# CVLAB-Unibo/MM2D3D

Hardware: AMD Instinct MI355X
Metric: LiDAR scenes/sec fwd+bwd (NuScenes ~35k pts, 5cm voxel) (higher is better)
Workload: dtype fp16 MFMA, fp32 accumulate, loss scale 65536 on the device (2D branch: IEEE fp16 maps and packed weights - the reference's precision: 16 = fp16 autocast + GradScaler) + f32 (3D sparse branch, fp32 as in the reference: f32 MFMA on narrow layers, fp32-faithful 3-term split-bf16 products with fp32 accu; 1 GPU; BASELINE.json configs[1]: NuScenes-shaped (32x1090 sweep, 34,880 pts/scene), 5 cm voxels, 480x302 RGB + sparse depth; full two-domain training step (train.py:186-292): 2D+3D fwd on source and target, 2 CE + 4 KL, backward, AdamW x2 + OneCycle; distinct_batches_rotated=4, parallelism=dp1

## Files before the change

include/mm2d3d.h:

```cpp
#ifndef MM2D3D_H
#define MM2D3D_H

#include <stddef.h>
#include <stdint.h>

#ifdef __cplusplus
extern "C" {
#endif

typedef void* mm_stream_t;

#define MM_OK 0
#define MM_ERR_ARG (-1)
#define MM_ERR_HIP (-2)
#define MM_ERR_WORKSPACE (-3)
#define MM_ERR_UNSUPPORTED (-4)

const char* mm_last_error(void);

typedef void* mm_handle_t;
size_t mm_handle_sync_bytes(void);
size_t mm_handle_fault_bytes(void);
int mm_create(int device_id, void* sync_dev, size_t sync_bytes, void* fault_host, size_t fault_bytes, mm_handle_t* out);
int mm_destroy(mm_handle_t h);
// ... 233 lines not shown
int mm_rmsprop_step(float* p, const float* g, float* sq, float* gavg, float* buf, int64_t n, double lr, double alpha, double eps,
                    double weight_decay, double momentum, double grad_scale, const int* skip_dev, int nskip, mm_stream_t stream);
int mm_sgd_prepare(const float* scale_dev, const int* found_dev, int nfound, int64_t* step_dev, int advance, double lr,
                   double momentum, double dampening, double weight_decay, double grad_scale, void* coef_dev, mm_stream_t stream);
int mm_adam_prepare(const float* scale_dev, const int* found_dev, int nfound, int64_t* step_dev, int advance, double lr,
                    double beta1, double beta2, double eps, double weight_decay, int decoupled, double grad_scale, void* coef_dev,
                    mm_stream_t stream);
int mm_rmsprop_prepare(const float* scale_dev, const int* found_dev, int nfound, int64_t* step_dev, int advance, double lr,
                       double alpha, double eps, double weight_decay, double momentum, double grad_scale, void* coef_dev,
                       mm_stream_t stream);
int mm_sgd_step_dev(float* p, const float* g, float* buf, int64_t n, int nesterov, const void* coef_dev, mm_stream_t stream);
int mm_adam_step_dev(float* p, const float* g, float* m, float* v, float* vmax, int64_t n, int decoupled, const void* coef_dev,
                     mm_stream_t stream);
int mm_rmsprop_step_dev(float* p, const float* g, float* sq, float* gavg, float* buf, int64_t n, const void* coef_dev,
                        mm_stream_t stream);

int mm_ema_row_bytes(void);
int mm_ema_update(const void* table_dev, int nrows, int64_t nblocks, double decay, int warmup, int64_t t_host, const int64_t* step_dev,
                  const void* coef_dev, const int* skip_dev, int nskip, mm_stream_t stream);
int mm_ema_swap(const void* table_dev, int nrows, int64_t nblocks, mm_stream_t stream);

size_t mm_grad_sqnorm_ws_bytes(int64_t n);
int mm_grad_sqnorm(const float* g, int64_t n, void* partial_ws, int64_t slot, int* found_dev, mm_stream_t stream);
int mm_clip_finalize(const void* partial_ws, const int64_t* counts, int narenas, const float* scale_dev, double grad_scale,
                     double max_norm, float* norm_out_dev, float* eff_scale_out_dev, mm_stream_t stream);
int mm_grad_clip_value(float* g, int64_t n, double clip_value, const float* scale_dev, double grad_scale, mm_stream_t stream);

int mm_conv2d_gemm(const void* A, int B, int Hi, int Wi, int Ca, int lda, void* O, int Ho, int Wo, int Cn, int ldo,
                   int out_f32, int Hg, int Wg, int so, int ooy, int oox, int sa, int fr, int ntaps, const int* ty,
                   const int* tx, const void* Wp, int nz, int64_t wz, int zpar, const float* bias, float* stats,
                   int64_t split_m, const void* addend, int ld_add, mm_stream_t stream);
int mm_conv2d_dgrad_s2(const void* dY, int B, int Ho, int Wo, int Cout, int ldy, void* dX, int H, int W, int Cin, int ldx, const void* Wd,
                       int k, int pad, const void* addend, int ld_add, mm_stream_t stream);
int64_t mm_conv2d_gemm_stat_rows(int64_t M, int nz);
int64_t mm_conv2d_3x3s1_stat_rows(int B, int H, int W);
int mm_conv2d_3x3s1(const void* A, int B, int H, int W, int Ca, int lda, void* O, int Cn, int ldo, const void* Wp,
                    const float* bias, int flip, float* stats, int split_b, mm_stream_t stream);
int mm_conv2d_3x3s1_pair(const void* A0, const void* A1, int B, int H, int W, int Ca, int lda, void* O0, void* O1, int Cn, int ldo,
                         const void* Wp0, const void* Wp1, int flip, float* stats0, float* stats1, int split_b, mm_stream_t stream);
size_t mm_conv2d_wgrad_ws_bytes(int64_t M, int Cn, int Ck, int ntaps);
int mm_conv2d_wgrad(const void* X, int B, int Hi, int Wi, int Ck, int ldx, const void* dY, int Hg, int Wg, int Cn,
                    int ldy, int sa, int ntaps, const int* ty, const int* tx, float* dW, int64_t sn, int64_t st,
                    int64_t sk, int accumulate, void* ws, size_t ws_bytes, mm_stream_t stream);
int mm_conv2d_wgrad3x3_pair(const void* X0, const void* X1, int B, int H, int W, int Ck, int ldx, const void* dY0, const void* dY1, int Cn,
                            int ldy, float* dW0, float* dW1, int64_t sn, int64_t st, int64_t sk, int accumulate, void* ws, size_t ws_bytes,
                            mm_stream_t stream);
int mm_conv2d_wgrad_slabs(const void* X, int B, int Hi, int Wi, int Ck, int ldx, const void* dY, int Hg, int Wg, int Cn, int ldy,
                          int sa, int ntaps, const int* ty, const int* tx, void* slabs, size_t slab_bytes, int* nsplit,
                          mm_stream_t stream);
int mm_conv2d_wgrad3x3_pair_slabs(const void* X0, const void* X1, int B, int H, int W, int Ck, int ldx, const void* dY0, const void* dY1,
                                  int Cn, int ldy, void* slabs, size_t slab_bytes, int* nsplit, mm_stream_t stream);
int mm_conv2d_wgrad_reduce_desc_bytes(void);
int64_t mm_conv2d_wgrad_reduce_blocks(int Cn, int Ck, int pair);
int mm_conv2d_wgrad_reduce_batch(const void* descs_dev, int n, int64_t total_blocks, mm_stream_t stream);
int64_t mm_conv2d_stem7_stat_rows(int B, int H, int W);
int mm_conv2d_stem7(const void* xb, int B, int Hb, int Wb, int H, int W, int R, int T, void* O, int ldo, const void* Wp, float* stats,
                    int split_b, mm_stream_t stream);
int mm_stem_prep(const float* in, int B, int C, int H, int W, int pad, int Hb, int Wb, int R, void* out, mm_stream_t stream);
int mm_pack_weights_bf16(const float* in, void* out, int Z, int N, int T, int K, int64_t sz, int64_t sn, int64_t st,
                         int64_t sk, mm_stream_t stream);
int mm_pack_weights_bf16_batch(const int64_t* desc, int ndesc, int64_t total_blocks, mm_stream_t stream);

size_t mm_bn2d_ws_bytes(int C);
int mm_bn2d_fwd_train(mm_handle_t h, const void* x, int ld_x, const void* res, int ld_r, int64_t N, int64_t Ns, int C, const float* weight,
                      const float* bias, float* running_mean, float* running_var, int64_t* num_batches_tracked, float eps,
                      float momentum, int relu, void* y, int ld_y, float* save_mean, float* save_invstd, void* ws,
// ... 31 lines not shown
                int ld_dx, void* dres, int ld_dr, float* dweight, float* dbias, int accumulate, void* ws, size_t ws_bytes,
                mm_stream_t stream);

int mm_colsum_bf16(const void* x, int ld_x, int64_t N, int C, float* out, int accumulate, void* ws, size_t ws_bytes,
                   mm_stream_t stream);

int mm_copy_rows_bf16(const void* src, int64_t ld_s, void* dst, int64_t ld_d, int64_t N, int C, mm_stream_t stream);
int mm_concat_bf16(void* const* parts, const int* channels, int nparts, void* wide, int64_t N, int split, mm_stream_t stream);
int mm_maxpool3x3s2_fwd(const void* x, int ldx, int B, int H, int W, int C, void* y, void* idx, mm_stream_t stream);
int mm_maxpool3x3s2_bwd(const void* dy, int ld_dy, const void* dy2, int ld_dy2, const void* idx, int B, int H, int W, int C, void* dx,
                        mm_stream_t stream);
size_t mm_head_ws_bytes(int B, int h, int w, int Hp, int Wp, int C, int NJ);
int mm_head_fwd(const void* x, int B, int Hp, int Wp, int ld, int h, int w, int C, const float* Wj, const float* bias,
                int NJ, float* out, void* ws, size_t ws_bytes, mm_stream_t stream);
int mm_head_bwd(const void* x, int B, int Hp, int Wp, int ld, int h, int w, int C, const float* Wj, int NJ,
                const float* dout, void* dx, float* dWj, void* ws, size_t ws_bytes, mm_stream_t stream);

int mm_conv2d_f32(const float* A, int B, int Hi, int Wi, int Ca, int ldA, float* O, int Ho, int Wo, int Cn, int ldO, int KH, int KW,
                  int so, int sgn, int off, int up, const float* W, int64_t w_sn, int64_t w_sc, int64_t w_sy, int64_t w_sx,
                  const float* bias, mm_stream_t stream);
size_t mm_conv2d_f32_wgrad_ws_bytes(int64_t n_pixels, int Cg, int Ca, int KH, int KW);
int mm_conv2d_f32_wgrad(const float* G, int B, int Hg, int Wg, int Cg, int ldG, const float* A, int Hi, int Wi, int Ca, int ldA,
                        int KH, int KW, int so, int sgn, int off, int up, float* dW, int64_t w_sn, int64_t w_sc, int64_t w_sy,
                        int64_t w_sx, int accumulate, void* ws, size_t ws_bytes, mm_stream_t stream);
int mm_colsum_f32(const float* x, int ld, int64_t N, int C, float* out, int accumulate, mm_stream_t stream);


int mm_conv2d_gemm_f16(const void* A, int B, int Hi, int Wi, int Ca, int lda, void* O, int Ho, int Wo, int Cn, int ldo,
                   int out_f32, int Hg, int Wg, int so, int ooy, int oox, int sa, int fr, int ntaps, const int* ty,
                   const int* tx, const void* Wp, int nz, int64_t wz, int zpar, const float* bias, float* stats,
                   int64_t split_m, const void* addend, int ld_add, mm_stream_t stream);
int mm_conv2d_dgrad_s2_f16(const void* dY, int B, int Ho, int Wo, int Cout, int ldy, void* dX, int H, int W, int Cin, int ldx, const void* Wd,
                       int k, int pad, const void* addend, int ld_add, mm_stream_t stream);
int64_t mm_conv2d_gemm_stat_rows_f16(int64_t M, int nz);
int64_t mm_conv2d_3x3s1_stat_rows_f16(int B, int H, int W);
int mm_conv2d_3x3s1_f16(const void* A, int B, int H, int W, int Ca, int lda, void* O, int Cn, int ldo, const void* Wp,
                    const float* bias, int flip, float* stats, int split_b, mm_stream_t stream);
int mm_conv2d_3x3s1_pair_f16(const void* A0, const void* A1, int B, int H, int W, int Ca, int lda, void* O0, void* O1, int Cn, int ldo,
                         const void* Wp0, const void* Wp1, int flip, float* stats0, float* stats1, int split_b, mm_stream_t stream);
int mm_conv2d_wgrad3x3_pair_f16(const void* X0, const void* X1, int B, int H, int W, int Ck, int ldx, const void* dY0, const void* dY1, int Cn,
                            int ldy, float* dW0, float* dW1, int64_t sn, int64_t st, int64_t sk, int accumulate, void* ws, size_t ws_bytes,
                            mm_stream_t stream);
size_t mm_conv2d_wgrad_ws_bytes_f16(int64_t M, int Cn, int Ck, int ntaps);
int mm_conv2d_wgrad_f16(const void* X, int B, int Hi, int Wi, int Ck, int ldx, const void* dY, int Hg, int Wg, int Cn,
                    int ldy, int sa, int ntaps, const int* ty, const int* tx, float* dW, int64_t sn, int64_t st,
                    int64_t sk, int accumulate, void* ws, size_t ws_bytes, mm_stream_t stream);
int mm_conv2d_wgrad_slabs_f16(const void* X, int B, int Hi, int Wi, int Ck, int ldx, const void* dY, int Hg, int Wg, int Cn, int ldy,
                          int sa, int ntaps, const int* ty, const int* tx, void* slabs, size_t slab_bytes, int* nsplit,
                          mm_stream_t stream);
int mm_conv2d_wgrad3x3_pair_slabs_f16(const void* X0, const void* X1, int B, int H, int W, int Ck, int ldx, const void* dY0, const void* dY1,
                                  int Cn, int ldy, void* slabs, size_t slab_bytes, int* nsplit, mm_stream_t stream);
int mm_conv2d_wgrad_reduce_desc_bytes_f16(void);
int64_t mm_conv2d_wgrad_reduce_blocks_f16(int Cn, int Ck, int pair);
int mm_conv2d_wgrad_reduce_batch_f16(const void* descs_dev, int n, int64_t total_blocks, mm_stream_t stream);
int64_t mm_conv2d_stem7_stat_rows_f16(int B, int H, int W);
int mm_conv2d_stem7_f16(const void* xb, int B, int Hb, int Wb, int H, int W, int R, int T, void* O, int ldo, const void* Wp, float* stats,
                    int split_b, mm_stream_t stream);
int mm_stem_prep_f16(const float* in, int B, int C, int H, int W, int pad, int Hb, int Wb, int R, void* out, mm_stream_t stream);
int mm_pack_weights_f16(const float* in, void* out, int Z, int N, int T, int K, int64_t sz, int64_t sn, int64_t st,
                         int64_t sk, mm_stream_t stream);
int mm_pack_weights_f16_batch(const int64_t* desc, int ndesc, int64_t total_blocks, mm_stream_t stream);
size_t mm_bn2d_ws_bytes_f16(int C);
int mm_bn2d_fwd_train_f16(mm_handle_t h, const void* x, int ld_x, const void* res, int ld_r, int64_t N, int64_t Ns, int C, const float* weight,
                      const float* bias, float* running_mean, float* running_var, int64_t* num_batches_tracked, float eps,
                      float momentum, int relu, void* y, int ld_y, float* save_mean, float* save_invstd, void* ws,
                      size_t ws_bytes, mm_stream_t stream);
// ... 39 lines not shown
```

mm2d3d_amd/_lib.py:

```python
from __future__ import annotations

import contextlib
import ctypes as C
import os
import subprocess

import torch

_HERE = os.path.dirname(os.path.abspath(__file__))
LIB_PATH = os.environ.get("MM_LIB_PATH") or os.path.join(_HERE, "libmm2d3d_hip.so")
CSRC = os.path.join(_HERE, "csrc")

_lib = None

vp, i32, i64, sz, f32, f64 = C.c_void_p, C.c_int32, C.c_int64, C.c_size_t, C.c_float, C.c_double

_PROTOS = {
    "mm_last_error": (C.c_char_p, []),
    "mm_handle_sync_bytes": (sz, []),
    "mm_handle_fault_bytes": (sz, []),
    "mm_create": (i32, [i32, vp, sz, vp, sz, C.POINTER(vp)]),
    "mm_destroy": (i32, [vp]),
    "mm_set_option": (i32, [vp, i32, i32]),
    "mm_get_option": (i32, [vp, i32]),
# ... 80 lines not shown
    "mm_lift_index_ws_bytes": (sz, [i64]),
    "mm_lift_index": (i32, [vp, vp, i32, i64, i32, i32, i32, vp, vp, vp, vp, vp, sz, vp]),
    "mm_lift_gather_key": (i32, [vp, i64, i64, i64, i64, vp, i64, i32, i32, i32, vp, vp]),
    "mm_lift_scatter_key": (i32, [vp, i32, vp, vp, i64, i32, i32, i64, i64, i64, i64, vp, vp]),
    "mm_eval_confusion": (i32, [vp, i32, vp, i32, vp, i64, i32, i64, vp, vp]),
    "mm_pselab_predict": (i32, [vp, i32, vp, i32, i64, i32, vp, vp, vp, vp, vp, vp, vp]),
    "mm_teacher_labels": (i32, [vp, i32, vp, i32, i64, i32, i32, f32, i64, vp, vp, vp, vp, vp, vp]),
    "mm_pselab_refine_ws_bytes": (sz, [i32]),
    "mm_pselab_refine": (i32, [vp, vp, i64, i32, i64, vp, vp, sz, vp]),
    "mm_grad_nonfinite": (i32, [vp, i64, vp, vp]),
    "mm_amp_update": (i32, [vp, vp, vp, i32, f64, f64, i32, vp]),
    "mm_optim_coef_bytes": (i32, []),
    "mm_sgd_step": (i32, [vp, vp, vp, i64, f64, f64, f64, f64, i32, i64, f64, vp, i32, vp]),
    "mm_adam_step": (i32, [vp, vp, vp, vp, vp, i64, f64, f64, f64, f64, f64, i32, i64, f64, vp, i32, vp]),
    "mm_rmsprop_step": (i32, [vp, vp, vp, vp, vp, i64, f64, f64, f64, f64, f64, f64, vp, i32, vp]),
    "mm_sgd_prepare": (i32, [vp, vp, i32, vp, i32, f64, f64, f64, f64, f64, vp, vp]),
    "mm_adam_prepare": (i32, [vp, vp, i32, vp, i32, f64, f64, f64, f64, f64, i32, f64, vp, vp]),
    "mm_rmsprop_prepare": (i32, [vp, vp, i32, vp, i32, f64, f64, f64, f64, f64, f64, vp, vp]),
    "mm_sgd_step_dev": (i32, [vp, vp, vp, i64, i32, vp, vp]),
    "mm_adam_step_dev": (i32, [vp, vp, vp, vp, vp, i64, i32, vp, vp]),
    "mm_rmsprop_step_dev": (i32, [vp, vp, vp, vp, vp, i64, vp, vp]),
    "mm_ema_row_bytes": (i32, []),
    "mm_ema_update": (i32, [vp, i32, i64, f64, i32, i64, vp, vp, vp, i32, vp]),
    "mm_ema_swap": (i32, [vp, i32, i64, vp]),
    "mm_grad_sqnorm_ws_bytes": (sz, [i64]),
    "mm_grad_sqnorm": (i32, [vp, i64, vp, i64, vp, vp]),
    "mm_clip_finalize": (i32, [vp, vp, i32, vp, f64, f64, vp, vp, vp]),
    "mm_grad_clip_value": (i32, [vp, i64, f64, vp, f64, vp]),
    "mm_conv2d_gemm": (i32, [vp, i32, i32, i32, i32, i32, vp, i32, i32, i32, i32, i32, i32, i32, i32, i32, i32, i32, i32, i32, vp, vp,
                             vp, i32, i64, i32, vp, vp, i64, vp, i32, vp]),
    "mm_conv2d_3x3s1": (i32, [vp, i32, i32, i32, i32, i32, vp, i32, i32, vp, vp, i32, vp, i32, vp]),
    "mm_conv2d_3x3s1_pair": (i32, [vp, vp, i32, i32, i32, i32, i32, vp, vp, i32, i32, vp, vp, i32, vp, vp, i32, vp]),
    "mm_conv2d_dgrad_s2": (i32, [vp, i32, i32, i32, i32, i32, vp, i32, i32, i32, i32, vp, i32, i32, vp, i32, vp]),
    "mm_conv2d_gemm_stat_rows": (i64, [i64, i32]),
    "mm_conv2d_3x3s1_stat_rows": (i64, [i32, i32, i32]),
    "mm_conv2d_wgrad_ws_bytes": (sz, [i64, i32, i32, i32]),
    "mm_conv2d_wgrad": (i32, [vp, i32, i32, i32, i32, i32, vp, i32, i32, i32, i32, i32, i32, vp, vp, vp, i64, i64, i64, i32, vp, sz,
                              vp]),
    "mm_conv2d_wgrad3x3_pair": (i32, [vp, vp, i32, i32, i32, i32, i32, vp, vp, i32, i32, vp, vp, i64, i64, i64, i32, vp, sz, vp]),
    "mm_conv2d_wgrad_slabs": (i32, [vp, i32, i32, i32, i32, i32, vp, i32, i32, i32, i32, i32, i32, vp, vp, vp, sz, vp, vp]),
    "mm_conv2d_wgrad3x3_pair_slabs": (i32, [vp, vp, i32, i32, i32, i32, i32, vp, vp, i32, i32, vp, sz, vp, vp]),
    "mm_conv2d_wgrad_reduce_desc_bytes": (i32, []),
    "mm_conv2d_wgrad_reduce_blocks": (i64, [i32, i32, i32]),
    "mm_conv2d_wgrad_reduce_batch": (i32, [vp, i32, i64, vp]),
    "mm_conv2d_f32": (i32, [vp, i32, i32, i32, i32, i32, vp, i32, i32, i32, i32, i32, i32, i32, i32, i32, i32, vp, i64, i64, i64, i64, vp, vp]),
    "mm_conv2d_f32_wgrad_ws_bytes": (sz, [i64, i32, i32, i32, i32]),
    "mm_conv2d_f32_wgrad": (i32, [vp, i32, i32, i32, i32, i32, vp, i32, i32, i32, i32, i32, i32, i32, i32, i32, i32, vp, i64, i64, i64, i64,
                                  i32, vp, sz, vp]),
    "mm_colsum_f32": (i32, [vp, i32, i64, i32, vp, i32, vp]),
    "mm_pack_weights_bf16": (i32, [vp, vp, i32, i32, i32, i32, i64, i64, i64, i64, vp]),
    "mm_pack_weights_bf16_batch": (i32, [vp, i32, i64, vp]),
    "mm_conv2d_stem7_stat_rows": (i64, [i32, i32, i32]),
    "mm_conv2d_stem7": (i32, [vp, i32, i32, i32, i32, i32, i32, i32, vp, i32, vp, vp, i32, vp]),
    "mm_stem_prep": (i32, [vp, i32, i32, i32, i32, i32, i32, i32, i32, vp, vp]),
    "mm_bn2d_ws_bytes": (sz, [i32]),
    "mm_bn2d_fwd_train": (i32, [vp, vp, i32, vp, i32, i64, i64, i32, vp, vp, vp, vp, vp, f32, f32, i32, vp, i32, vp, vp, vp, sz, vp]),
    "mm_bn2d_single_launch": (i32, [vp, i64, i64, i32, i32]),
    "mm_bn2d_fwd_train_pre": (i32, [vp, i32, vp, i32, i64, i64, i32, vp, vp, vp, vp, vp, f32, f32, i32, vp, i32, vp, vp, vp, i64, vp, sz, vp]),
    "mm_bn2d_fwd_train_pre_pool": (i32, [vp, i32, i32, i32, i32, i32, i32, vp, vp, vp, vp, vp, f32, f32, vp, i32, vp, vp, vp, vp, vp, i64, vp, sz, vp]),
    "mm_bn2d_bwd_pool": (i32, [vp, i32, vp, i32, vp, i32, i32, i32, i32, vp, i32, i32, vp, vp, vp, vp, vp, i32, vp, vp, i32, vp, sz, vp]),
    "mm_bn2d_fwd_train_pair": (i32, [vp, vp, vp, i64, i64, i32, f32, f32, i32, vp, sz, vp]),
    "mm_bn2d_bwd_pair": (i32, [vp, vp, vp, i32, i64, i64, i32, i32, vp, sz, vp]),
    "mm_bn2d_fwd_eval": (i32, [vp, i32, vp, i32, i64, i32, vp, vp, vp, vp, f32, i32, vp, i32, vp]),
    "mm_bn2d_bwd": (i32, [vp, vp, i32, vp, i32, vp, i32, vp, i32, i32, i64, i64, i32, vp, vp, vp, vp, vp, i32, vp, i32, vp, vp, i32, vp, sz, vp]),
    "mm_colsum_bf16": (i32, [vp, i32, i64, i32, vp, i32, vp, sz, vp]),
    "mm_copy_rows_bf16": (i32, [vp, i64, vp, i64, i64, i32, vp]),
    "mm_concat_bf16": (i32, [vp, vp, i32, vp, i64, i32, vp]),
    "mm_maxpool3x3s2_fwd": (i32, [vp, i32, i32, i32, i32, i32, vp, vp, vp]),
    "mm_maxpool3x3s2_bwd": (i32, [vp, i32, vp, i32, vp, i32, i32, i32, i32, vp, vp]),
    "mm_head_ws_bytes": (sz, [i32, i32, i32, i32, i32, i32, i32]),
    "mm_head_fwd": (i32, [vp, i32, i32, i32, i32, i32, i32, i32, vp, vp, i32, vp, vp, sz, vp]),
    "mm_head_bwd": (i32, [vp, i32, i32, i32, i32, i32, i32, i32, vp, i32, vp, vp, vp, vp, sz, vp]),
}


class Bn2dFwdArgs(C.Structure):
    _fields_ = [("x", C.c_void_p), ("ld_x", C.c_int), ("res", C.c_void_p), ("ld_r", C.c_int), ("weight", C.c_void_p), ("bias", C.c_void_p),
                ("running_mean", C.c_void_p), ("running_var", C.c_void_p), ("num_batches_tracked", C.c_void_p), ("y", C.c_void_p),
                ("ld_y", C.c_int), ("save_mean", C.c_void_p), ("save_invstd", C.c_void_p)]


class Bn2dBwdArgs(C.Structure):
    _fields_ = [("x", C.c_void_p), ("ld_x", C.c_int), ("dy", C.c_void_p), ("ld_dy", C.c_int), ("dy2", C.c_void_p), ("ld_dy2", C.c_int),
                ("yout", C.c_void_p), ("ld_y", C.c_int), ("weight", C.c_void_p), ("bias", C.c_void_p), ("save_mean", C.c_void_p),
                ("save_invstd", C.c_void_p), ("dx", C.c_void_p), ("ld_dx", C.c_int), ("dres", C.c_void_p), ("ld_dr", C.c_int),
                ("dweight", C.c_void_p), ("dbias", C.c_void_p)]


class HipLibraryMissing(RuntimeError):
    pass


H16_2D = {
    "mm_conv2d_gemm": "mm_conv2d_gemm_f16",
    "mm_conv2d_dgrad_s2": "mm_conv2d_dgrad_s2_f16",
    "mm_conv2d_3x3s1": "mm_conv2d_3x3s1_f16",
    "mm_conv2d_3x3s1_pair": "mm_conv2d_3x3s1_pair_f16",
    "mm_conv2d_gemm_stat_rows": "mm_conv2d_gemm_stat_rows_f16",
    "mm_conv2d_3x3s1_stat_rows": "mm_conv2d_3x3s1_stat_rows_f16",
    "mm_bn2d_fwd_train_pre": "mm_bn2d_fwd_train_pre_f16",
    "mm_bn2d_single_launch": "mm_bn2d_single_launch_f16",
    "mm_bn2d_fwd_train_pair": "mm_bn2d_fwd_train_pair_f16",
    "mm_bn2d_fwd_train_pre_pool": "mm_bn2d_fwd_train_pre_pool_f16",
    "mm_bn2d_bwd_pool": "mm_bn2d_bwd_pool_f16",
    "mm_bn2d_bwd_pair": "mm_bn2d_bwd_pair_f16",
    "mm_conv2d_wgrad_ws_bytes": "mm_conv2d_wgrad_ws_bytes_f16",
    "mm_conv2d_wgrad": "mm_conv2d_wgrad_f16",
    "mm_conv2d_wgrad3x3_pair": "mm_conv2d_wgrad3x3_pair_f16",
    "mm_conv2d_wgrad_slabs": "mm_conv2d_wgrad_slabs_f16",
    "mm_conv2d_wgrad3x3_pair_slabs": "mm_conv2d_wgrad3x3_pair_slabs_f16",
    "mm_conv2d_wgrad_reduce_desc_bytes": "mm_conv2d_wgrad_reduce_desc_bytes_f16",
    "mm_conv2d_wgrad_reduce_blocks": "mm_conv2d_wgrad_reduce_blocks_f16",
    "mm_conv2d_wgrad_reduce_batch": "mm_conv2d_wgrad_reduce_batch_f16",
    "mm_stem_prep": "mm_stem_prep_f16",
    "mm_conv2d_stem7_stat_rows": "mm_conv2d_stem7_stat_rows_f16",
    "mm_conv2d_stem7": "mm_conv2d_stem7_f16",
    "mm_pack_weights_bf16": "mm_pack_weights_f16",
    "mm_pack_weights_bf16_batch": "mm_pack_weights_f16_batch",
    "mm_bn2d_ws_bytes": "mm_bn2d_ws_bytes_f16",
    "mm_bn2d_fwd_train": "mm_bn2d_fwd_train_f16",
    "mm_bn2d_fwd_eval": "mm_bn2d_fwd_eval_f16",
    "mm_bn2d_bwd": "mm_bn2d_bwd_f16",
    "mm_colsum_bf16": "mm_colsum_f16",
    "mm_maxpool3x3s2_fwd": "mm_maxpool3x3s2_fwd_f16",
    "mm_maxpool3x3s2_bwd": "mm_maxpool3x3s2_bwd_f16",
    "mm_head_ws_bytes": "mm_head_ws_bytes_f16",
    "mm_head_fwd": "mm_head_fwd_f16",
    "mm_head_bwd": "mm_head_bwd_f16",
}
for _a, _b in H16_2D.items():
# ... 206 lines not shown
```

mm2d3d_amd/conv2d.py:

```python
from __future__ import annotations

import ctypes as C
import os
import weakref

import torch

from . import _lib, domains, gradsink
from ._lib import check, ptr, stream

CL = torch.channels_last

WHOLE_ITEMS = [2 if os.environ.get("MM_CONV_WHOLE_ITEMS", "0") != "0" else 0]
LEGACY3X3 = [{"1": 4, "2": 8, "3": 12}.get(os.environ.get("MM_CONV3X3_LEGACY", "0"), 0)]
BN_PRE = [{"0": False, "1": True}.get(os.environ.get("MM_BN2D_PRE", "auto"), "auto")]
WGRAD_BATCH = [os.environ.get("MM_CONV_WGRAD_BATCH", "1") != "0"]
WGRAD_BATCH_GRAPH = [os.environ.get("MM_CONV_WGRAD_BATCH_GRAPH", "1") != "0"]
STEM7 = [os.environ.get("MM_CONV_STEM7", "1") != "0"]
DGRAD_S2 = [os.environ.get("MM_CONV_DGRAD_S2", "1") != "0"]
PAIR = [os.environ.get("MM_CONV_PAIR", "1") != "0"]
PAIR_WGRAD = [os.environ.get("MM_CONV_PAIR_WGRAD", "1") != "0"]

HALF = [torch.float16]


def set_half(dtype):
    if dtype not in (torch.bfloat16, torch.float16):
        raise ValueError("the 16-bit storage format of the 2D branch is torch.bfloat16 or torch.float16")
    HALF[0] = dtype


class _Lib2d:

    def __getattr__(self, name):
        L = _lib.lib()
        if HALF[0] == torch.float16:
            alt = _lib.H16_2D.get(name)
            if alt is not None:
                return getattr(L, alt)
        return getattr(L, name)


_LIB2D = _Lib2d()


def lib2d():
    return _LIB2D


def nhwc_pitch(x):
    if x.dtype != HALF[0]:
        x = x.to(HALF[0])
    B, C, H, W = x.shape
    s0, s1, s2, s3 = x.stride()
    if s1 == 1 and s3 >= C and s3 % 8 == 0 and s2 == W * s3 and s0 == H * W * s3 and x.data_ptr() % 16 == 0:
        return x, s3
    return x.contiguous(memory_format=CL), C


def _arr(v):
    return (C.c_int * len(v))(*v)


def as_nhwc_bf16(x):
    if x.dtype != HALF[0]:
        x = x.to(HALF[0])
    if not x.is_contiguous(memory_format=CL):
        x = x.contiguous(memory_format=CL)
# ... 535 lines not shown
```

mm2d3d_amd/csrc/conv2d.hip:

```cpp
#include <hip/hip_bf16.h>

#include <type_traits>

#include "common.h"
#include "h16.h"

typedef h16x8 bf16x8;
typedef short s16x4 __attribute__((ext_vector_type(4)));
typedef float f32x16 __attribute__((ext_vector_type(16)));

namespace {

constexpr int MAXT = 16;

struct ConvP {
  const u16* A;
  int B, Hi, Wi, Ca, lda;
  void* O;
  int Ho, Wo, Cn, ldo;
  int Hg, Wg;
  int so, ooy, oox;
  int sa, fr;
  int ntaps;
  short ty[MAXT], tx[MAXT];
// ... 295 lines not shown
    }
#pragma unroll
    for (int j = 0; j < TN; j++) {
#pragma unroll
      for (int q = 0; q < 4; q++) {
        const int n = n0 + wn * (BN / 2) + j * 32 + 8 * q + 4 * fh;
        if (n >= p.Cn) continue;
        float v[4];
#pragma unroll
        for (int e = 0; e < 4; e++) v[e] = acc[i][j][4 * q + e];
        if (vec) {
          if (p.bias) {
            const float4 bb = *(const float4*)&p.bias[n];
            v[0] += bb.x, v[1] += bb.y, v[2] += bb.z, v[3] += bb.w;
          }
          if (p.out_f32) {
            *(float4*)&((float*)p.O)[orow * p.ldo + n] = make_float4(v[0], v[1], v[2], v[3]);
          } else {
            uint2 o;
            o.x = (unsigned)f2bf(v[0]) | ((unsigned)f2bf(v[1]) << 16);
            o.y = (unsigned)f2bf(v[2]) | ((unsigned)f2bf(v[3]) << 16);
            *(uint2*)&((u16*)p.O)[orow * p.ldo + n] = o;
          }
        } else {
#pragma unroll
          for (int e = 0; e < 4; e++)
            if (n + e < p.Cn) {
              const float w = v[e] + (p.bias ? p.bias[n + e] : 0.f);
              if (p.out_f32)
                ((float*)p.O)[orow * p.ldo + n + e] = w;
              else
                ((u16*)p.O)[orow * p.ldo + n + e] = f2bf(w);
            }
        }
      }
    }
  }
}

struct C3P {
  const u16* A;
  int B, H, W, Ca, lda;
  u16* O;
  int Cn, ldo;
  const u16* Wp;
  const float* bias;
  int flip;
  int whole;
  int legacy;
  float* stats;
  int split_b;
  int tiles_y, tiles_x;
  int B1;
  const u16* A1;
  u16* O1;
  const u16* Wp1;
  float* stats1;
};
#define MM_DIAG(p, bit) ((DIAG & (bit)) != 0)

__device__ __attribute__((aligned(16))) unsigned int g_dump[256];


#ifdef MM_DIAG_CLOCK
__device__ unsigned long long g_clk[3][1024][2];
#define MM_CLK_BEGIN() const unsigned long long clk_t0 = __builtin_amdgcn_s_memtime(), clk_r0 = __builtin_amdgcn_s_memrealtime()
// ... 1975 lines not shown
    const int sy = y + r - pad, sx = x - pad;
    v[sl] = (r < R && sy >= 0 && sy < H && sx >= 0 && sx < W) ? f2bf(in[((int64_t)(b * C + c) * H + sy) * W + sx]) : (u16)0;
  }
  unsigned w[4];
#pragma unroll
  for (int i = 0; i < 4; i++) w[i] = (unsigned)v[2 * i] | ((unsigned)v[2 * i + 1] << 16);
  *(uint4*)(out + (int64_t)gid * 8) = make_uint4(w[0], w[1], w[2], w[3]);
}

int fill_taps(ConvP* p, const int* ty, const int* tx, int nt) {
  if (nt > MAXT) return -1;
  p->ntaps = nt;
  p->wtaps = nt;
  p->zwin = 0;
  for (int i = 0; i < nt; i++) {
    p->ty[i] = (short)ty[i];
    p->tx[i] = (short)tx[i];
    p->wt[i] = (short)i;
  }
  for (int i = 0; i < 4; i++) p->zt0[i] = p->znt[i] = 0;
  return 0;
}

}

extern "C" {

#ifdef MM_DIAG_CLOCK
int MM_SYM(mm_diag_clock_read)(void* out_host, size_t bytes) {
  return hipMemcpyFromSymbol(out_host, HIP_SYMBOL(g_clk), bytes < sizeof(g_clk) ? bytes : sizeof(g_clk)) == hipSuccess ? 0 : -1;
}
#endif

static int gemm_launch(ConvP p, int nz, int steps_max, hipStream_t s) {
  const int B = p.B, Hg = p.Hg, Wg = p.Wg, Cn = p.Cn;
  const int64_t M = (int64_t)B * Hg * Wg;
  if (M == 0) return MM_OK;
  MM_CHECK_ARG(M < (1ll << 31), "conv2d_gemm: too many output pixels for 32-bit pixel indices");
  {
    constexpr int single_max = 4;
    p.nbuf = (steps_max <= single_max && (Cn <= 64 || steps_max == 1)) ? 1 : 2;
  }
  if (Cn <= 64) {
    size_t lds = (size_t)p.nbuf * (128 * 64 + 64 * 64) * 2;
    hipLaunchKernelGGL(k_conv_gemm<64>, dim3((unsigned)mm_cdiv(M, 128), (unsigned)mm_cdiv(Cn, 64), nz), dim3(256), lds, s, p);
  } else {
    size_t lds = (size_t)p.nbuf * (128 * 64 + 128 * 64) * 2;
    static unsigned once = 0;
    if (mm_attr_todo(&once)) {
      MM_HIP(hipFuncSetAttribute((const void*)k_conv_gemm<128>, hipFuncAttributeMaxDynamicSharedMemorySize, (int)(2 * (128 * 64 + 128 * 64) * 2)));
      mm_attr_done(&once);
    }
    hipLaunchKernelGGL(k_conv_gemm<128>, dim3((unsigned)mm_cdiv(M, 128), (unsigned)mm_cdiv(Cn, 128), nz), dim3(256), lds, s, p);
  }
  MM_LAUNCH_CHECK();
  return MM_OK;
}

int MM_SYM(mm_conv2d_gemm)(const void* A, int B, int Hi, int Wi, int Ca, int lda, void* O, int Ho, int Wo, int Cn, int ldo,
                   int out_f32, int Hg, int Wg, int so, int ooy, int oox, int sa, int fr, int ntaps, const int* ty,
                   const int* tx, const void* Wp, int nz, int64_t wz, int zpar, const float* bias, float* stats, int64_t split_m,
                   const void* addend, int ld_add, hipStream_t s) {
  MM_CHECK_ARG(Ca % 64 == 0 && lda % 8 == 0 && ((uintptr_t)A % 16) == 0 && ((uintptr_t)Wp % 16) == 0,
               "conv2d_gemm: Ca must be a multiple of 64 and pointers 16-B aligned (Ca=%d lda=%d)", Ca, lda);
  MM_CHECK_ARG(!stats || (!out_f32 && Cn % 32 == 0 && ldo % 8 == 0 && ((uintptr_t)O % 16) == 0 && ((uintptr_t)bias % 16) == 0),
               "conv2d_gemm: statistics need a 16-bit output, Cn a multiple of 32, ldo of 8");
  MM_CHECK_ARG(!addend || (!out_f32 && Cn % 8 == 0 && ldo % 8 == 0 && ld_add % 8 == 0 && ((uintptr_t)O % 16) == 0 && ((uintptr_t)addend % 16) == 0 &&
                           ((uintptr_t)bias % 16) == 0),
               "conv2d_gemm: an addend needs a 16-bit output, channels and pitches multiples of 8, 16-byte aligned maps");
  MM_CHECK_ARG(fr == 1 || fr == 2, "conv2d_gemm: fr must be 1 or 2");
  ConvP p;
// ... 437 lines not shown
```

Before: 486.1 scenes/s.

## Add persistent weight-resident conv GEMM kernel with double-buffered activation tiles

Adds a persistent-grid conv GEMM kernel that loads the whole packed weight matrix into LDS once per workgroup and then loops over 128-row output tiles. Activation chunks are double-buffered with global_load_lds, and the next tile's first chunk is prefetched during the epilogue. It also folds the four transposed-conv sub-positions into one wide N tile and handles the stride-2 1x1 dgrad zero fill inside the same kernel. The path is on by default for eligible shapes. It trades higher LDS use, and possibly lower occupancy, for fewer weight reloads and fewer launch tails.

```diff
diff --git a/include/mm2d3d.h b/include/mm2d3d.h
--- a/include/mm2d3d.h
+++ b/include/mm2d3d.h
@@ -289,6 +289,7 @@
                    int64_t split_m, const void* addend, int ld_add, mm_stream_t stream);
 int mm_conv2d_dgrad_s2(const void* dY, int B, int Ho, int Wo, int Cout, int ldy, void* dX, int H, int W, int Cin, int ldx, const void* Wd,
                        int k, int pad, const void* addend, int ld_add, mm_stream_t stream);
+int mm_conv2d_gemm_rw(int mode, int wgs);
 int64_t mm_conv2d_gemm_stat_rows(int64_t M, int nz);
 int64_t mm_conv2d_3x3s1_stat_rows(int B, int H, int W);
 int mm_conv2d_3x3s1(const void* A, int B, int H, int W, int Ca, int lda, void* O, int Cn, int ldo, const void* Wp,
@@ -386,6 +387,7 @@
                    int64_t split_m, const void* addend, int ld_add, mm_stream_t stream);
 int mm_conv2d_dgrad_s2_f16(const void* dY, int B, int Ho, int Wo, int Cout, int ldy, void* dX, int H, int W, int Cin, int ldx, const void* Wd,
                        int k, int pad, const void* addend, int ld_add, mm_stream_t stream);
+int mm_conv2d_gemm_rw_f16(int mode, int wgs);
 int64_t mm_conv2d_gemm_stat_rows_f16(int64_t M, int nz);
 int64_t mm_conv2d_3x3s1_stat_rows_f16(int B, int H, int W);
 int mm_conv2d_3x3s1_f16(const void* A, int B, int H, int W, int Ca, int lda, void* O, int Cn, int ldo, const void* Wp,
diff --git a/mm2d3d_amd/_lib.py b/mm2d3d_amd/_lib.py
--- a/mm2d3d_amd/_lib.py
+++ b/mm2d3d_amd/_lib.py
@@ -136,6 +136,7 @@
     "mm_conv2d_3x3s1": (i32, [vp, i32, i32, i32, i32, i32, vp, i32, i32, vp, vp, i32, vp, i32, vp]),
     "mm_conv2d_3x3s1_pair": (i32, [vp, vp, i32, i32, i32, i32, i32, vp, vp, i32, i32, vp, vp, i32, vp, vp, i32, vp]),
     "mm_conv2d_dgrad_s2": (i32, [vp, i32, i32, i32, i32, i32, vp, i32, i32, i32, i32, vp, i32, i32, vp, i32, vp]),
+    "mm_conv2d_gemm_rw": (i32, [i32, i32]),
     "mm_conv2d_gemm_stat_rows": (i64, [i64, i32]),
     "mm_conv2d_3x3s1_stat_rows": (i64, [i32, i32, i32]),
     "mm_conv2d_wgrad_ws_bytes": (sz, [i64, i32, i32, i32]),
@@ -200,6 +201,7 @@
     "mm_conv2d_dgrad_s2": "mm_conv2d_dgrad_s2_f16",
     "mm_conv2d_3x3s1": "mm_conv2d_3x3s1_f16",
     "mm_conv2d_3x3s1_pair": "mm_conv2d_3x3s1_pair_f16",
+    "mm_conv2d_gemm_rw": "mm_conv2d_gemm_rw_f16",
     "mm_conv2d_gemm_stat_rows": "mm_conv2d_gemm_stat_rows_f16",
     "mm_conv2d_3x3s1_stat_rows": "mm_conv2d_3x3s1_stat_rows_f16",
     "mm_bn2d_fwd_train_pre": "mm_bn2d_fwd_train_pre_f16",
diff --git a/mm2d3d_amd/conv2d.py b/mm2d3d_amd/conv2d.py
--- a/mm2d3d_amd/conv2d.py
+++ b/mm2d3d_amd/conv2d.py
@@ -30,10 +30,26 @@
     HALF[0] = dtype
 
 
+GEMM_RW = [(1 if os.environ.get("MM_CONV_GEMM_RW", "1") != "0" else 0) | (2 if os.environ.get("MM_CONV_GEMM_RW_DEBUG", "0") != "0" else 0), 0]
+_GEMM_RW_SENT = [False]
+
+
+def set_gemm_rw(mode, wgs=0):
+    prev = tuple(GEMM_RW)
+    GEMM_RW[0], GEMM_RW[1] = int(mode), int(wgs)
+    L = _lib.lib()
+    check(L.mm_conv2d_gemm_rw(GEMM_RW[0], GEMM_RW[1]), "conv2d_gemm_rw")
+    check(L.mm_conv2d_gemm_rw_f16(GEMM_RW[0], GEMM_RW[1]), "conv2d_gemm_rw")
+    _GEMM_RW_SENT[0] = True
+    return prev
+
+
 class _Lib2d:
 
     def __getattr__(self, name):
         L = _lib.lib()
+        if not _GEMM_RW_SENT[0]:
+            set_gemm_rw(*GEMM_RW)
         if HALF[0] == torch.float16:
             alt = _lib.H16_2D.get(name)
             if alt is not None:
diff --git a/mm2d3d_amd/csrc/conv2d.hip b/mm2d3d_amd/csrc/conv2d.hip
--- a/mm2d3d_amd/csrc/conv2d.hip
+++ b/mm2d3d_amd/csrc/conv2d.hip
@@ -351,6 +351,254 @@
               else
                 ((u16*)p.O)[orow * p.ldo + n + e] = f2bf(w);
             }
+        }
+      }
+    }
+  }
+}
+
+struct RwP {
+  ConvP c;
+  int fold;
+  int dz;
+  int steps;
+  int ntiles;
+  int tyx[8];
+};
+
+template <int TN>
+__global__ __launch_bounds__(256, 2) void k_conv_gemm_rw(RwP q) {
+  const ConvP& p = q.c;
+  extern __shared__ __attribute__((aligned(16))) u16 smem[];
+  constexpr int NT = TN * 64;
+  u16* Bs = smem;
+  u16* As = smem + q.steps * NT * 64;
+  float* Bias = (float*)(As + 2 * 128 * 64);
+  const int tid = threadIdx.x, wave = tid >> 6, lane = tid & 63;
+  const int wm = wave >> 1, wn = wave & 1;
+  const int64_t M = (int64_t)p.B * p.Hg * p.Wg;
+  const int cc = tid & 7, r0 = tid >> 3;
+  const int kcn = p.Ca >> 6;
+
+  for (int s = 0; s < q.steps; s++) {
+    const int tl = s / kcn, kc = s - tl * kcn;
+    const int woff = p.wt[tl] * p.Ca + kc * 64;
+#pragma unroll
+    for (int i = 0; i < NT / 32; i++) {
+      const int row = r0 + 32 * i;
+      const u16* g = p.W + (int64_t)row * p.wtaps * p.Ca + woff + ((cc ^ ((row >> 1) & 7)) << 3);
+      __builtin_amdgcn_global_load_lds((const __attribute__((address_space(1))) void*)g,
+                                       (__attribute__((address_space(3))) void*)(Bs + s * NT * 64 + (wave * 8 + 32 * i) * 64), 16, 0, 0);
+    }
+  }
+
+  const u16* abase[4];
+  unsigned amask[4];
+  auto decode = [&](int tile) {
+    const int64_t m0 = (int64_t)tile * 128;
+#pragma unroll
+    for (int i = 0; i < 4; i++) {
+      const int row = r0 + 32 * i;
+      const int64_t m = m0 + row;
+      int ab = -1, ay = 0, ax = 0;
+      if (m < M) {
+        const unsigned mu = (unsigned)m, t = mu / (unsigned)p.Wg;
+        ax = (int)(mu - t * (unsigned)p.Wg);
+        ab = (int)(t / (unsigned)p.Hg);
+        ay = (int)(t - (unsigned)ab * (unsigned)p.Hg);
+      }
+      abase[i] = p.A + ((int64_t)((ab < 0 ? 0 : ab) * p.Hi + ay * p.sa) * p.Wi + ax * p.sa) * p.lda + ((cc ^ ((row >> 1) & 7)) << 3);
+      unsigned mk = 0;
+      if (ab >= 0)
+        for (int t = 0; t < p.ntaps; t++) {
+          const int v = q.tyx[t];
+          const int sy = ay * p.sa + (short)(v & 0xffff), sx = ax * p.sa + (v >> 16);
+          if (sy >= 0 && sx >= 0 && sy < p.Hi && sx < p.Wi) mk |= 1u << t;
+        }
+      amask[i] = mk;
+    }
+  };
+  auto issue = [&](int s, int buf) {
+    const int tap = s / kcn, kc = s - tap * kcn;
+    const int v = q.tyx[tap];
+    const int64_t toff = ((int64_t)(short)(v & 0xffff) * p.Wi + (v >> 16)) * p.lda + kc * 64;
+#pragma unroll
+    for (int i = 0; i < 4; i++) {
+      const u16* g = (amask[i] >> tap) & 1u ? abase[i] + toff : (const u16*)g_zero16;
+      __builtin_amdgcn_global_load_lds((const __attribute__((address_space(1))) void*)g,
+                                       (__attribute__((address_space(3))) void*)(As + buf * 128 * 64 + (wave * 8 + 32 * i) * 64), 16, 0, 0);
+    }
+  };
+
+  const int fr_ = lane & 31, fh = lane >> 5;
+  const int schunk = frag_chunk(lane);
+  const bool remap = p.so != 1 || p.Ho != p.Hg || p.Wo != p.Wg;
+  int tile = blockIdx.x;
+  if (tile >= q.ntiles) return;
+  decode(tile);
+  issue(0, 0);
+  if (p.bias && tid < NT) Bias[tid] = p.bias[q.fold ? tid & 63 : tid];
+  __syncthreads();
+  unsigned g = 0;
+  constexpr int NST = 4 * TN;
+  bool stores_behind = false;
+  for (; tile < q.ntiles; tile += gridDim.x) {
+    f32x16 acc[2][TN];
+#pragma unroll
+    for (int i = 0; i < 2; i++)
+#pragma unroll
+      for (int j = 0; j < TN; j++)
+#pragma unroll
+        for (int r = 0; r < 16; r++) acc[i][j][r] = 0.f;
+
+    for (int s = 0; s < q.steps; s++, g++) {
+      const int buf = g & 1;
+      if (s == 0 && stores_behind)
+        asm volatile("s_waitcnt vmcnt(%0)\n\ts_barrier" ::"n"(NST) : "memory");
+      else
+        asm volatile("s_waitcnt vmcnt(0)\n\ts_barrier" ::: "memory");
+      if (s + 1 < q.steps) {
+        issue(s + 1, buf ^ 1);
+      } else if (tile + (int)gridDim.x < q.ntiles) {
+        decode(tile + gridDim.x);
+        issue(0, buf ^ 1);
+      }
+      const u16* Ab = As + buf * 128 * 64;
+      const u16* Bb = Bs + s * NT * 64;
+#pragma unroll
+      for (int kk = 0; kk < 4; kk++) {
+        bf16x8 af[2], bf[TN];
+        const int ch = kk * 2 + fh;
+#pragma unroll
+        for (int i = 0; i < 2; i++) {
+          int row = wm * 64 + i * 32 + fr_;
+          af[i] = *(const bf16x8*)&Ab[row * 64 + ((ch ^ ((row >> 1) & 7)) << 3)];
+        }
+#pragma unroll
+        for (int j = 0; j < TN; j++) {
+          int row = wn * (NT / 2) + j * 32 + fr_;
+          bf[j] = *(const bf16x8*)&Bb[row * 64 + ((ch ^ ((row >> 1) & 7)) << 3)];
+        }
+#pragma unroll
+        for (int i = 0; i < 2; i++)
+#pragma unroll
+          for (int j = 0; j < TN; j++) acc[i][j] = MM_MFMA_32x32x16(bf[j], af[i], acc[i][j]);
+      }
+    }
+
+    const int64_t m0 = (int64_t)tile * 128;
+    stores_behind = m0 + 128 <= M;
+    int ora[2], orb[2], mra[2], mrb[2];
+#pragma unroll
+    for (int i = 0; i < 2; i++) {
+      mra[i] = (int)m0 + wm * 64 + i * 32 + (lane & 15), mrb[i] = mra[i] + 16;
+      auto out_row = [&](int m) -> int {
+        if (remap) {
+          const unsigned mu = (unsigned)m, t = mu / (unsigned)p.Wg;
+          const int gx = (int)(mu - t * (unsigned)p.Wg);
+          const int b = (int)(t / (unsigned)p.Hg), gy = (int)(t - (unsigned)b * (unsigned)p.Hg);
+          return (b * p.Ho + gy * p.so) * p.Wo + gx * p.so;
+        }
+        return m;
+      };
+      ora[i] = mra[i] < M ? out_row(mra[i]) : -1;
+      orb[i] = mrb[i] < M ? out_row(mrb[i]) : -1;
+    }
+#pragma unroll
+    for (int j = 0; j < TN; j++) {
+      uint4 sxa[2], sxb[2];
+      const int ntot = wn * (NT / 2) + j * 32;
+      const int zf = q.fold ? ntot >> 6 : 0;
+      const int nf = q.fold ? ntot & 63 : ntot;
+      const int zoff = (zf >> 1) * p.Wo + (zf & 1);
+      const int64_t ssub = ((int64_t)zf * q.ntiles + tile) * 2 + wm;
+      typedef float f32x4 __attribute__((ext_vector_type(4)));
+      f32x4 bq[4] = {};
+      const unsigned ba = (unsigned)(uintptr_t)(__attribute__((address_space(3))) float*)&Bias[ntot + 4 * fh];
+      if (TN < 4 && p.bias) {
+        asm volatile("ds_read_b128 %0, %4\n\tds_read_b128 %1, %4 offset:32\n\tds_read_b128 %2, %4 offset:64\n\tds_read_b128 %3, %4 offset:96\n\t"
+                     "s_waitcnt lgkmcnt(0)"
+                     : "=&v"(bq[0]), "=&v"(bq[1]), "=&v"(bq[2]), "=&v"(bq[3])
+                     : "v"(ba));
+      }
+      constexpr bool ADD = TN < 4;
+      uint4 ada[2], adb[2];
+      if (ADD && p.addend) {
+#pragma unroll
+        for (int i = 0; i < 2; i++) {
+          ada[i] = *(const uint4*)(p.addend + (ora[i] >= 0 ? (int64_t)(ora[i] + zoff) * p.ld_add : 0) + nf + 8 * schunk);
+          adb[i] = *(const uint4*)(p.addend + (orb[i] >= 0 ? (int64_t)(orb[i] + zoff) * p.ld_add : 0) + nf + 8 * schunk);
+        }
+      }
+#pragma unroll
+      for (int i = 0; i < 2; i++) {
+        unsigned D[4][2];
+#pragma unroll
+        for (int qd = 0; qd < 4; qd++) {
+          float v[4];
+#pragma unroll
+          for (int e = 0; e < 4; e++) v[e] = acc[i][j][4 * qd + e];
+          if (p.bias) {
+            f32x4 bb;
+            if constexpr (TN < 4) bb = bq[qd];
+            else asm volatile("ds_read_b128 %0, %1\n\ts_waitcnt lgkmcnt(0)" : "=v"(bb) : "v"(ba + 32 * qd));
+            v[0] += bb.x, v[1] += bb.y, v[2] += bb.z, v[3] += bb.w;
+          }
+          D[qd][0] = (unsigned)f2bf(v[0]) | ((unsigned)f2bf(v[1]) << 16);
+          D[qd][1] = (unsigned)f2bf(v[2]) | ((unsigned)f2bf(v[3]) << 16);
+        }
+        uint4 xa, xb;
+        frag_rows(D, xa, xb);
+        const int n = nf + 8 * schunk;
+        u16* rowa = ora[i] >= 0 ? (u16*)p.O + (int64_t)(ora[i] + zoff) * p.ldo : nullptr;
+        u16* rowb = orb[i] >= 0 ? (u16*)p.O + (int64_t)(orb[i] + zoff) * p.ldo : nullptr;
+        if (ADD && p.addend) {
+          if (rowa) xa = add_h8(xa, ada[i]);
+          if (rowb) xb = add_h8(xb, adb[i]);
+        }
+        sxa[i] = xa, sxb[i] = xb;
+        if (rowa) *(uint4*)(rowa + n) = xa;
+        if (rowb) *(uint4*)(rowb + n) = xb;
+      }
+      if (p.stats) {
+#pragma unroll
+        for (int grp = 0; grp < 2; grp++) {
+          float st[16];
+#pragma unroll
+          for (int t = 0; t < 16; t++) st[t] = 0.f;
+#pragma unroll
+          for (int i = 0; i < 2; i++) {
+            stats_accum(sxa[i], ora[i] >= 0 && (mra[i] < p.split_m) == (grp == 0), st);
+            stats_accum(sxb[i], orb[i] >= 0 && (mrb[i] < p.split_m) == (grp == 0), st);
+          }
+          stats_store(p.stats, 2 * ssub + grp, p.Cn, nf, lane, row_reduce_scatter16(st, lane & 15), false);
+        }
+      }
+    }
+    if (TN < 4 && q.dz) {
+      for (int z = 1; z < 4; z++) {
+        const int zoff = (z >> 1) * p.Wo + (z & 1);
+#pragma unroll
+        for (int j = 0; j < TN; j++) {
+          const int n = wn * (NT / 2) + j * 32 + 8 * schunk;
+          uint4 ada[2], adb[2];
+          if (p.addend) {
+#pragma unroll
+            for (int i = 0; i < 2; i++) {
+              ada[i] = *(const uint4*)(p.addend + (ora[i] >= 0 ? (int64_t)(ora[i] + zoff) * p.ld_add : 0) + n);
+              adb[i] = *(const uint4*)(p.addend + (orb[i] >= 0 ? (int64_t)(orb[i] + zoff) * p.ld_add : 0) + n);
+            }
+          }
+#pragma unroll
+          for (int i = 0; i < 2; i++) {
+            uint4 xa = make_uint4(0u, 0u, 0u, 0u), xb = xa;
+            if (p.addend) {
+              xa = add_h8(xa, ada[i]);
+              xb = add_h8(xb, adb[i]);
+            }
+            if (ora[i] >= 0) *(uint4*)((u16*)p.O + (int64_t)(ora[i] + zoff) * p.ldo + n) = xa;
+            if (orb[i] >= 0) *(uint4*)((u16*)p.O + (int64_t)(orb[i] + zoff) * p.ldo + n) = xb;
+          }
         }
       }
     }
@@ -2392,11 +2640,93 @@
 }
 #endif
 
+static int g_rw_mode = 1, g_rw_wgs = 0;
+int MM_SYM(mm_conv2d_gemm_rw)(int mode, int wgs) {
+  MM_CHECK_ARG(mode >= 0 && mode < 8 && wgs >= 0, "conv2d_gemm_rw: mode is 0..7, wgs >= 0");
+  __atomic_store_n(&g_rw_mode, mode, __ATOMIC_RELAXED);
+  __atomic_store_n(&g_rw_wgs, wgs, __ATOMIC_RELAXED);
+  return MM_OK;
+}
+
+static int rw_launch(const ConvP& p, int nz, hipStream_t s, int* done) {
+  *done = 0;
+  const int mode = __atomic_load_n(&g_rw_mode, __ATOMIC_RELAXED), wgs_forced = __atomic_load_n(&g_rw_wgs, __ATOMIC_RELAXED);
+  if (!(mode & 1)) return MM_OK;
+  const int64_t M = (int64_t)p.B * p.Hg * p.Wg;
+  RwP q;
+  q.c = p;
+  q.fold = q.dz = 0;
+  int nt_eff = p.ntaps;
+  if (nz == 4 && p.zpar && !p.zwin) {
+    if (p.ntaps != 1 || p.Cn != 64 || p.wz != (int64_t)p.Cn * p.Ca || p.so != 2) return MM_OK;
+    q.fold = 1;
+  } else if (nz == 4 && p.zpar && p.zwin) {
+    if (p.znt[0] != 1 || p.zt0[0] != 0 || p.znt[1] || p.znt[2] || p.znt[3] || p.ntaps != 1 || p.so != 2 || p.Cn > 128) return MM_OK;
+    q.dz = 1;
+    nt_eff = 1;
+  } else if (nz != 1 || p.zwin) {
+    return MM_OK;
+  }
+  const int NT = q.fold ? 4 * p.Cn : p.Cn;
+  q.steps = nt_eff * (p.Ca / 64);
+  if (p.out_f32 || p.fr != 1 || p.ooy || p.oox || (p.Cn & 63) || (p.ldo & 7) || p.lda < p.Ca || p.ldo < p.Cn || ((uintptr_t)p.O & 15) ||
+      ((uintptr_t)p.bias & 15) || (p.addend && ((p.ld_add & 7) || p.ld_add < p.Cn || ((uintptr_t)p.addend & 15))))
+    return MM_OK;
+  if ((NT != 64 && NT != 128 && NT != 256) || q.steps < 1 || (int64_t)NT * q.steps * 64 > 32768) return MM_OK;
+  if (NT == 256 && p.addend) return MM_OK;
+  if ((int64_t)p.B * p.Hi * p.Wi >= (1ll << 31) || (int64_t)p.B * p.Ho * p.Wo >= (1ll << 31)) return MM_OK;
+  q.ntiles = (int)mm_cdiv(M, 128);
+  static const int ncu = [] {
+    int dev = 0, n = 0;
+    if (hipGetDevice(&dev) != hipSuccess || hipDeviceGetAttribute(&n, hipDeviceAttributeMultiprocessorCount, dev) != hipSuccess || n <= 0) n = 256;
+    return n;
+  }();
+  for (int t = 0; t < 8; t++) q.tyx[t] = t < p.ntaps ? (int)(((unsigned)p.ty[t] & 0xffffu) | ((unsigned)p.tx[t] << 16)) : 0;
+  const size_t lds = ((size_t)q.steps * NT * 64 + 2 * 128 * 64) * 2 + (size_t)NT * 4;
+  const int per_cu = lds <= 66560 ? 2 : 1;
+  if (wgs_forced <= 0 && !(mode & 4) && per_cu == 1 && !q.fold) return MM_OK;
+  int wgs = wgs_forced > 0 ? wgs_forced : per_cu * ncu;
+  if (wgs > q.ntiles) wgs = q.ntiles;
+  for (int e = 0; e < 2; e++) {
+    const int64_t m = e ? M - 1 : 0;
+    const int ax = (int)(m % p.Wg), ay = (int)(m / p.Wg % p.Hg), ab = (int)(m / p.Wg / p.Hg);
+    for (int t = 0; t < nt_eff; t++) {
+      const int sy = ay * p.sa + p.ty[t], sx = ax * p.sa + p.tx[t];
+      if (sy < 0 || sx < 0 || sy >= p.Hi || sx >= p.Wi) continue;
+      const int64_t px = ((int64_t)ab * p.Hi + sy) * p.Wi + sx;
+      MM_CHECK_ARG(ab >= 0 && ab < p.B && px >= 0 && px < (int64_t)p.B * p.Hi * p.Wi, "conv2d_gemm_rw: a source pixel outside the input map");
+    }
+  }
+  static unsigned once = 0;
+  if (mm_attr_todo(&once)) {
+    const int mx = (32768 + 2 * 128 * 64) * 2 + 256 * 4;
+    MM_HIP(hipFuncSetAttribute((const void*)k_conv_gemm_rw<1>, hipFuncAttributeMaxDynamicSharedMemorySize, mx));
+    MM_HIP(hipFuncSetAttribute((const void*)k_conv_gemm_rw<2>, hipFuncAttributeMaxDynamicSharedMemorySize, mx));
+    MM_HIP(hipFuncSetAttribute((const void*)k_conv_gemm_rw<4>, hipFuncAttributeMaxDynamicSharedMemorySize, mx));
+    mm_attr_done(&once);
+  }
+  if (mode & 2)
+    fprintf(stderr, "conv2d_gemm_rw: K=%d N=%d %s M=%lld tiles=%d wgs=%d lds=%zu addend=%d stats=%d\n", q.steps * 64, NT,
+            q.fold ? "convT-fwd" : q.dz ? "dgrad-s2-1x1" : p.sa == 2 ? "gather-s2" : "plain", (long long)M, q.ntiles, wgs, lds,
+            p.addend != nullptr, p.stats != nullptr);
+  if (NT == 64) hipLaunchKernelGGL(k_conv_gemm_rw<1>, dim3((unsigned)wgs), dim3(256), lds, s, q);
+  else if (NT == 128) hipLaunchKernelGGL(k_conv_gemm_rw<2>, dim3((unsigned)wgs), dim3(256), lds, s, q);
+  else hipLaunchKernelGGL(k_conv_gemm_rw<4>, dim3((unsigned)wgs), dim3(256), lds, s, q);
+  *done = 1;
+  MM_LAUNCH_CHECK();
+  return MM_OK;
+}
+
 static int gemm_launch(ConvP p, int nz, int steps_max, hipStream_t s) {
   const int B = p.B, Hg = p.Hg, Wg = p.Wg, Cn = p.Cn;
   const int64_t M = (int64_t)B * Hg * Wg;
   if (M == 0) return MM_OK;
   MM_CHECK_ARG(M < (1ll << 31), "conv2d_gemm: too many output pixels for 32-bit pixel indices");
+  {
+    int done = 0;
+    const int r = rw_launch(p, nz, s, &done);
+    if (done || r != MM_OK) return r;
+  }
   {
     constexpr int single_max = 4;
     p.nbuf = (steps_max <= single_max && (Cn <= 64 || steps_max == 1)) ? 1 : 2;
```

Result: no change. 488.1 scenes/s, median of 6 (+0.4%).
